# jimonld2000/AudioDenoiser

Measured on AMD Instinct MI355X. Metric: spectrogram frames/sec (forward), 513x256 fp32, higher is better.
Workload: dtype f32; 1 GPU; BASELINE configs[1]: batch=64 synthetic 513x256 fp32 spectrograms on one MI355X, full U-Net forward + per-clip perceptual loss; batch_per_gpu=64, global_batch=64, freq_bins=513, frames=256, parallelism=clips sharded over 1 rank(s), weights replicated, no data-path collective, lib_digest=fdf05542d610

## Files before the change

### audiodenoiser_amd/csrc/adn_internal.h

```cpp
#pragma once
#include <hip/hip_runtime.h>
#include <cstddef>
#include <cstdint>

namespace adn {

template <typename T> constexpr int ACT_BLOCK = 32 / (int)sizeof(T);
template <typename T>
__host__ __device__ __forceinline__ long act_off(int C, long HW, long pix, int c)
{
    constexpr int B = ACT_BLOCK<T>;
    (void)C;
    return ((long)(c / B) * HW + pix) * B + (c % B);
}

#ifdef __HIPCC__
constexpr unsigned ADN_DMA_OOB = 0xfffffff0u;
__device__ __forceinline__ void dma16_buf(__amdgpu_buffer_rsrc_t rsrc, unsigned voff, unsigned soff, float *lds_wave_base)
{
    __builtin_amdgcn_raw_ptr_buffer_load_lds(rsrc, (__attribute__((address_space(3))) void *)lds_wave_base, 16, voff, soff, 0, 0);
}
__device__ __forceinline__ __amdgpu_buffer_rsrc_t dma_rsrc(const void *base, unsigned bytes)
{
    return __builtin_amdgcn_make_buffer_rsrc(const_cast<void *>(base), 0, bytes, 0x00020000);
// ... 50 lines not shown
    void *pool;
    int N, H, W;
    int Cout;
    int tilesY, tilesX, nct;
    int pair;
    FastDiv fdGc, fdNcg, fdTx, fdTy;
    int nwg_total;
    int split;
    int ksplit;
    int nwg_base;
    float *partial;
    const float *dotw;
    float *dot_out;
    float dot_bias;
    const float *firstw, *firstb;
};

inline bool wino4_pair_mode(const ConvArgs &a)
{
    if (a.W > 16) return false;
    const size_t i0 = (size_t)a.s0.C * a.s0.H * a.s0.W * 4, i1 = (size_t)a.s1.C * a.s1.H * a.s1.W * 4;
    return (i0 > i1 ? i0 : i1) + (size_t)a.H * a.W * 32 < (size_t)0xfffffff0u;
}

constexpr int ADN_MAX_KSPLIT = 8;

inline long conv_workgroups(const ConvArgs &a) { return (long)a.N * a.tilesY * a.tilesX * a.nct; }

inline int wino_ksplit(long nwg, int nchunk)
{
// ... 23 lines not shown
        }
    }
    return best;
}

inline int conv16_ksplit(long nwg, int nchunk, size_t out_floats)
{
    if (nwg > 64) return 1;
    int ks = 1;
    while (ks < 8 && nwg * ks * 2 <= 256 && nchunk % (ks * 2) == 0 && nchunk / (ks * 2) >= 4 &&
           (size_t)(ks * 2) * out_floats * 4 <= ((size_t)32 << 20))
        ks *= 2;
    return ks;
}

enum ConvKind { CONV3X3_RELU = 0, CONV3X3_RELU_POOL = 1, CONVT2X2 = 2, CONV3X3_RELU_DOT = 3 };

struct ConvGeom {
    int TH;
    int BN;
    int KC;
};
ConvGeom conv_geom(ConvKind kind, int Cout, bool f16);
long conv_mfma_tiles(ConvKind kind, bool f16, ConvArgs &a);

hipError_t launch_conv_mfma(ConvKind kind, const ConvArgs &a, bool f16, hipStream_t st);
hipError_t launch_conv_reduce_f16(ConvKind kind, const float *partial, const float *bias, void *out, void *pool, int ksplit, int N,
                                  int H, int W, int Cout, hipStream_t st);
hipError_t launch_convt_reduce(const float *partial, const float *bias, float *out, int ksplit, int N, int Ho, int Wo, int Cout,
                               hipStream_t st);
constexpr int WINO_BN = 32;
hipError_t launch_wino_conv(ConvKind kind, const ConvArgs &a, hipStream_t st);
long wino_tiles(ConvArgs &a);
hipError_t launch_wino_reduce(ConvKind kind, const ConvArgs &a, hipStream_t st);
bool wino4_applicable(ConvKind kind, const ConvArgs &a, bool force);
long wino4_workgroups(const ConvArgs &a);
hipError_t launch_wino4_conv(ConvKind kind, const ConvArgs &a, hipStream_t st);

bool conv16_applicable(ConvKind kind, const ConvArgs &a);
hipError_t launch_conv16(ConvKind kind, const ConvArgs &a, bool resident, hipStream_t st);

bool convt16_applicable(const ConvArgs &a);
hipError_t launch_convt16(const ConvArgs &a, hipStream_t st);

hipError_t launch_conv_first(const float *x, const float *w9x64, const float *bias, void *out, bool f16,
                             int N, int H, int W, int Cin, hipStream_t st);
hipError_t launch_dot_finish(const float *planes, int nplanes, float bias, float *y, long npix, hipStream_t st);
hipError_t launch_conv_out(const void *in, bool f16, const float *w64, float bias, float *out, long npix, long HW,
                           long out_stride, hipStream_t st);
hipError_t launch_nhwc_to_nchw(const void *in, bool f16, float *out, int N, int H, int W, int C, hipStream_t st);

hipError_t launch_stft_mag(const float *audio, int n_clips, long L, int n_fft, int hop, int center, long n_frames,
// ... 76 lines not shown
```

### audiodenoiser_amd/csrc/conv_kernels.hip

```cpp
#include "adn_internal.h"

#include <atomic>
#include <cstdlib>

namespace adn {

typedef float f32x16 __attribute__((ext_vector_type(16)));
typedef float f32x4 __attribute__((ext_vector_type(4)));
typedef _Float16 f16x8 __attribute__((ext_vector_type(8)));
typedef _Float16 f16x4 __attribute__((ext_vector_type(4)));

namespace {

constexpr int TW = 16;
constexpr int CONVT_KG = 2, CONVT_WPE = 4;

template <typename T> struct Elem;
template <> struct Elem<float> { static constexpr int EPV = 4; };
template <> struct Elem<_Float16> { static constexpr int EPV = 8; };

__device__ __forceinline__ int xcd_remap(int b, int nwg)
{
    const int xcd = b & 7, q = nwg >> 3, r = nwg & 7;
    const int start = xcd < r ? xcd * (q + 1) : r * (q + 1) + (xcd - r) * q;
// ... 249 lines not shown
template <> struct Piece<_Float16> { typedef f16x8 type; };

template <typename T, int TH, int BN, int WM, int WN, int EPI, int HALVES = 1>
__device__ __forceinline__ void conv_epilogue_staged(const ConvArgs &p, f32x16 (&acc)[TH * TW / 32 / WM][BN / 32 / WN],
                                                     const float (&bias_r)[BN / 32 / WN], float *smem, int tid, int lane,
                                                     int wave, int ct, int n, int ty, int tx)
{
    constexpr int MB = TH * TW / 32 / WM, NB = BN / 32 / WN, NT = 64 * WM * WN;
    constexpr int EPP = 16 / sizeof(T);
    constexpr int RS = BN + EPP;
    constexpr int NPIX = TH * TW, PPR = BN / EPP;
    typedef typename Piece<T>::type piece_t;
    const int wm = wave / WN, wn = wave % WN;
    const int hh = lane >> 5, l31 = lane & 31;
    T *stage = reinterpret_cast<T *>(smem);
    static_assert(HALVES == 1 || (EPI == CONVT2X2 && HALVES == 2 && WM == 2 && TH % 2 == 0), "two-half staging: convT, WM = 2");

#pragma unroll
    for (int hf = 0; hf < HALVES; ++hf) {
    if (HALVES == 1 || wm == hf) {
#pragma unroll
    for (int j = 0; j < NB; ++j) {
        const int col = (wn * NB + j) * 32 + l31;
        const float bv = bias_r[j];
#pragma unroll
        for (int i = 0; i < MB; ++i) {
            const int pix0 = ((HALVES == 1 ? wm * MB : 0) + i) * 32 + 4 * hh;
            float v[16];
#pragma unroll
            for (int r = 0; r < 16; ++r) {
                v[r] = acc[i][j][r] + bv;
                if (EPI != CONVT2X2) v[r] = relu_nan(v[r]);
            }
            if constexpr (sizeof(T) == 4) {
#pragma unroll
                for (int r = 0; r < 16; ++r) stage[(pix0 + (r & 3) + 8 * (r >> 2)) * RS + col] = v[r];
            } else {
                const bool odd = l31 & 1;
#pragma unroll
                for (int r = 0; r < 16; r += 2) {
                    const float send = odd ? v[r] : v[r + 1];
                    const float recv = __shfl_xor(send, 1, 64);
                    const float lo = odd ? recv : v[r], hi = odd ? v[r + 1] : recv;
                    const int pix = pix0 + ((r + (odd ? 1 : 0)) & 3) + 8 * (r >> 2);
                    typedef _Float16 h2 __attribute__((ext_vector_type(2)));
                    *reinterpret_cast<h2 *>(stage + pix * RS + (col & ~1)) = h2{(_Float16)lo, (_Float16)hi};
                }
// ... 10 lines not shown
        const int Ho = 2 * p.H, Wo = 2 * p.W;
        const int ncg = p.Cout >> 6, di = ct / ncg, cg = ct - di * ncg;
        const size_t bstr = (size_t)Ho * Wo * BE;
        T *ob = outp + (size_t)n * Ho * Wo * p.Cout + (size_t)(NBLK * cg) * bstr;
        const int gxl = lane >> 2, dj = (lane >> 1) & 1, half = lane & 1;
        const int gx = tx * TW + gxl;
        constexpr int THH = TH / HALVES;
#pragma unroll
        for (int it = 0; it < NBLK * THH / (NT / 64); ++it) {
            const int run = it * (NT / 64) + wave;
            const int b8 = run / THH, py = run - b8 * THH;
            const int gy = ty * TH + hf * THH + py;
            const piece_t val = *reinterpret_cast<const piece_t *>(stage + (py * TW + gxl) * RS + dj * 64 + b8 * BE + half * EPP);
            if (gy < p.H && gx < p.W)
                *reinterpret_cast<piece_t *>(ob + b8 * bstr + ((size_t)(2 * gy + di) * Wo + 2 * gx + dj) * BE + half * EPP) = val;
        }
        if (HALVES > 1 && hf + 1 < HALVES) __syncthreads();
    } else if constexpr (EPI == CONV3X3_RELU_DOT) {
        static_assert(PPR <= 64 && (PPR & (PPR - 1)) == 0 && NT % PPR == 0, "pieces of a pixel must sit in one wave");
        float wv[EPP];
#pragma unroll
        for (int e = 0; e < EPP; ++e) wv[e] = p.dotw[(tid % PPR) * EPP + e];
#pragma unroll
        for (int it = 0; it < NPIX * PPR / NT; ++it) {
            const int id = it * NT + tid;
            const int pix = id / PPR, part = id - pix * PPR;
            const int gy = ty * TH + (pix >> 4), gx = tx * TW + (pix & 15);
            const piece_t val = *reinterpret_cast<const piece_t *>(stage + pix * RS + part * EPP);
            float s = 0.f;
#pragma unroll
// ... 55 lines not shown
    static constexpr int SLOTS = A_SLOTS + B_SLOTS;
    static constexpr int NPIECE = (SLOTS + NT - 1) / NT;
    static constexpr int A_ROUNDS = (A_SLOTS + NT - 1) / NT;
    static constexpr size_t LDS_BYTES = (size_t)2 * SLOTS * 16;
    static_assert(B_SLOTS % 64 == 0, "weight slab must be a whole number of wave copies");
};

typedef adn_bf16x8 bf16x8;

template <typename T, int TH, int BN, int WM, int WN, int TAPS, int KG, int EPI, int WPE, int SPLIT = 0, int KSPLIT = 0>
__global__ __launch_bounds__(64 * WM * WN, WPE) void conv_dma(const ConvArgs p)
{
    using C = DmaCfg<T, TH, BN, WM, WN, TAPS, KG, SPLIT>;
    static_assert(!KSPLIT || EPI == CONVT2X2 || (sizeof(T) == 2 && EPI == CONV3X3_RELU), "K split: transposed convolutions, fp16 3x3 layers");
    static_assert(!SPLIT || (sizeof(T) == 4 && KG == 2 && TAPS == 1), "SPLIT: fp32 storage, one 16-channel chunk (two fp32 k-groups), 1 tap");
    constexpr int NT = C::NT, EPV = Elem<T>::EPV, HALO = C::HALO, PW = C::PW;
    static_assert(2 * EPV == ACT_BLOCK<T>, "one k-group = one channel block of the activation layout");
    constexpr int PSLOT = C::PSLOT, RSLOT = C::RSLOT, A_SLOTS = C::A_SLOTS, SLOTS = C::SLOTS, NPIECE = C::NPIECE;
    constexpr int A_ROUNDS = C::A_ROUNDS;
    constexpr int B_DW = C::B_SLOTS * 4;
    constexpr int MB = TH * TW / 32 / WM, NB = BN / 32 / WN;
    static_assert(WM * WN == 4 || WM * WN == 8, "4 or 8 waves per workgroup");
    static_assert(MB >= 1 && NB >= 1, "tile too small");

    extern __shared__ __attribute__((aligned(16))) float smem[];

    const int tid = threadIdx.x;
    const int lane = tid & 63;
    const int wave = __builtin_amdgcn_readfirstlane(tid >> 6);
    const int wm = wave / WN, wn = wave % WN;
// ... 12 lines not shown
        ct = lid - q1 * p.nct;
        const int q2 = fastdiv(q1, p.fdTx.d, p.fdTx.m);
        tx = q1 - q2 * p.tilesX;
        n = fastdiv(q2, p.fdTy.d, p.fdTy.m);
        ty = q2 - n * p.tilesY;
    } else {
        ct = lid % p.nct;
        lid /= p.nct;
        tx = lid % p.tilesX;
        lid /= p.tilesX;
        ty = lid % p.tilesY;
        n = lid / p.tilesY;
    }
    const int gy0 = ty * TH - HALO, gx0 = tx * TW - HALO;

    auto src_base = [&](const ConvSrc &s) { return reinterpret_cast<const char *>(static_cast<const T *>(s.ptr) + (size_t)n * s.H * s.W * s.C); };
    const char *hptr = src_base(p.s0);
    const __amdgpu_buffer_rsrc_t wrs = dma_rsrc(static_cast<const float *>(p.wpk) + (size_t)ct * p.nchunk * B_DW,
                                                (unsigned)((size_t)p.nchunk * B_DW * 4));
    unsigned cstr = (unsigned)((size_t)KG * p.s0.H * p.s0.W * ACT_BLOCK<T> * sizeof(T));
    unsigned wsoff = 0;
    const int c0 = KSPLIT ? ksp * nloc : 0;
    bool in2 = false;
    if constexpr (KSPLIT) {
        wsoff = (unsigned)c0 * (unsigned)(B_DW * 4);
        if (c0 > p.nchunk0) {
            in2 = true;
            cstr = (unsigned)((size_t)KG * p.s1.H * p.s1.W * ACT_BLOCK<T> * sizeof(T));
            hptr = src_base(p.s1) + (size_t)(c0 - p.nchunk0) * cstr;
        } else {
            hptr += (size_t)c0 * cstr;
        }
    }
    const unsigned loff = lane * 16;
    unsigned hcur[A_ROUNDS];
// ... 6 lines not shown
        } else if (want_b) {
            dma16_buf(wrs, loff, wsoff + (unsigned)(sb - A_SLOTS) * 16u, dst);
        }
    };
#pragma unroll
    for (int k = 0; k < NPIECE; ++k) dma_piece(k, 0, false, true);

    auto plan = [&](const ConvSrc &src) {
#pragma unroll
        for (int r = 0; r < A_ROUNDS; ++r) {
            const int s = r * NT + tid;
            const int row = s / RSLOT, k = s - row * RSLOT;
            const int pix = k / PSLOT, q = k - pix * PSLOT;
            const bool data = s < C::A_USED && pix < PW && q < C::KQ;
            const int y0 = gy0 + row - src.offY, x0 = gx0 + pix - src.offX;
            hcur[r] = (data && y0 >= 0 && y0 < src.H && x0 >= 0 && x0 < src.W)
                          ? (unsigned)act_off<T>(src.C, (long)src.H * src.W, y0 * src.W + x0, q * EPV) * (unsigned)sizeof(T) : ADN_DMA_OOB;
        }
    };
    if (in2) plan(p.s1);
    else plan(p.s0);

    auto dma_chunk = [&](int c, int buf, bool with_b = true) {
        if (c == p.nchunk0) {
            hptr = src_base(p.s1);
            cstr = (unsigned)((size_t)KG * p.s1.H * p.s1.W * ACT_BLOCK<T> * sizeof(T));
            plan(p.s1);
        }
#pragma unroll
        for (int k = 0; k < NPIECE; ++k) dma_piece(k, buf, true, with_b);
        hptr += cstr;
        wsoff += B_DW * 4;
    };

    float bias_r[NB];
#pragma unroll
    for (int j = 0; j < NB; ++j) bias_r[j] = p.bias[ct * BN + (wn * NB + j) * 32 + l31];

    f32x16 acc[MB][NB];
#pragma unroll
    for (int i = 0; i < MB; ++i)
#pragma unroll
        for (int j = 0; j < NB; ++j)
#pragma unroll
            for (int r = 0; r < 16; ++r) acc[i][j][r] = 0.f;

    const int a_lane = ((wm * MB * 2 + ((lane >> 4) & 1)) * RSLOT + (lane & 15) * PSLOT) * 4 + hh * 4;
    const int b_lane = A_SLOTS * 4 + hh * BN * 4 + (wn * NB * 32 + l31) * 4;

    dma_chunk(c0, 0, false);
    asm volatile("s_waitcnt vmcnt(0)" ::: "memory");
    __syncthreads();
// ... 46 lines not shown
                } else {
#pragma unroll
                    for (int i = 0; i < MB; ++i)
#pragma unroll
                        for (int j = 0; j < NB; ++j)
                            acc[i][j] = __builtin_amdgcn_mfma_f32_32x32x16_f16(__builtin_bit_cast(f16x8, a[i]),
                                                                               __builtin_bit_cast(f16x8, b[j]), acc[i][j], 0, 0, 0);
                }
            }
        }
        asm volatile("s_waitcnt vmcnt(0)" ::: "memory");
        __syncthreads();
    }
    if constexpr (KSPLIT && EPI != CONVT2X2) {
        conv_epilogue_raw<TH, BN, WM, WN>(p, acc, lane, wave, ct, n + ksp * p.N, ty, tx);
    } else if constexpr (sizeof(T) == 2 || EPI == CONVT2X2) {
        constexpr size_t tile = (size_t)TH * TW * (BN + 16 / sizeof(T)) * sizeof(T);
        constexpr int HALVES = tile <= C::LDS_BYTES ? 1 : 2;
        static_assert(tile / HALVES <= C::LDS_BYTES, "staging tile (or half of it) must fit the two images");
        conv_epilogue_staged<T, TH, BN, WM, WN, EPI, HALVES>(p, acc, bias_r, smem, tid, lane, wave, ct, KSPLIT ? n + ksp * p.N : n, ty, tx);
    } else {
        conv_epilogue<T, TH, BN, WM, WN, EPI>(p, acc, bias_r, lane, wave, ct, n, ty, tx);
    }
}

constexpr int FIRST_ROWS = 8;

template <typename T>
__global__ __launch_bounds__(256) void conv_first_kernel(const float *__restrict__ x, const float *__restrict__ w9x64,
                                                         const float *__restrict__ bias, T *__restrict__ out,
                                                         int H, int W, int tiles_y, int tiles_x, int cols, int Cin)
// ... 280 lines not shown

long conv_mfma_tiles(ConvKind kind, bool f16, ConvArgs &a)
{
    const ConvGeom g = conv_geom(kind, a.Cout, f16);
    a.tilesY = (a.H + g.TH - 1) / g.TH;
    a.tilesX = (a.W + TW - 1) / TW;
    a.nct = (kind == CONVT2X2 ? 4 * a.Cout : a.Cout) / g.BN;
    return conv_workgroups(a);
}

hipError_t launch_conv_mfma(ConvKind kind, const ConvArgs &a, bool f16, hipStream_t st)
{
    return f16 ? launch_conv_mfma_t<_Float16>(kind, a, st) : launch_conv_mfma_t<float>(kind, a, st);
}

hipError_t launch_conv_reduce_f16(ConvKind kind, const float *partial, const float *bias, void *out, void *pool, int ksplit, int N,
                                  int H, int W, int Cout, hipStream_t st)
{
    const bool pl = kind == CONV3X3_RELU_POOL;
    const long items = pl ? (long)N * ((H + 1) / 2) * ((W + 1) / 2) * (Cout / 4) : (long)N * H * W * (Cout / 4);
    const long blocks = (items + 255) / 256;
    if (ksplit < 2 || ksplit > ADN_MAX_KSPLIT || (Cout & 15) || (kind != CONV3X3_RELU && !pl) || (pl && !pool) || blocks <= 0 || blocks > 0x7fffffffL)
        return hipErrorInvalidValue;
    if (pl)
        hipLaunchKernelGGL(conv_reduce_f16_kernel<true>, dim3((unsigned)blocks), dim3(256), 0, st, partial, bias,
                           static_cast<_Float16 *>(out), static_cast<_Float16 *>(pool), ksplit, N, H, W, Cout);
    else
        hipLaunchKernelGGL(conv_reduce_f16_kernel<false>, dim3((unsigned)blocks), dim3(256), 0, st, partial, bias,
                           static_cast<_Float16 *>(out), static_cast<_Float16 *>(nullptr), ksplit, N, H, W, Cout);
    return hipGetLastError();
// ... 77 lines not shown
```

### audiodenoiser_amd/csrc/unet.hip

```cpp
#include "adn_host.h"

#include <algorithm>
#include <cmath>
#include <cstdlib>
#include <cstring>
#include <memory>
#include <vector>

using adn::aligned_to;
using adn::DeviceGuard;
using adn::fail;
using adn::fail_hip;

namespace {

constexpr float BN_EPS = 1e-5f;
constexpr int CH[5] = {64, 128, 256, 512, 1024};

enum LayerKind { CONV3, CONVT };
struct LayerDesc {
    LayerKind kind;
    int level;
    int C0, C1;
    int Cout;
// ... 14 lines not shown
        t.v[t.n++] = LayerDesc{CONVT, l + 1, CH[l + 1], 0, CH[l]};
        t.v[t.n++] = LayerDesc{CONV3, l, CH[l], CH[l], CH[l]};
        t.v[t.n++] = LayerDesc{CONV3, l, CH[l], 0, CH[l]};
    }
    return t;
}
constexpr LayerTable NET = make_layers();
static_assert(NET.n == N_LAYERS && NET.v[0].Cout == 64 && NET.v[8].C0 == 1024 && NET.v[9].kind == CONVT && NET.v[N_LAYERS - 1].Cout == 64,
              "layer table: 9 layers down to the bottleneck, then 4 x (convT, conv, conv)");
static_assert(6 * (1 + N_CONV3) + 2 * N_CONVT + 2 == ADN_N_WEIGHT_TENSORS, "layer table does not match the weight tensor list");
static_assert(1 + N_LAYERS + 1 == ADN_N_LAUNCHES, "layer table does not match the timing slots");

struct LayerWeights {
    size_t w_off, b_off;
    size_t w4_off;
    size_t w16_off;
    size_t braw_off;
};

}

struct adn_unet {
    int device = 0;
    float *dev = nullptr;
    size_t dev_floats = 0;
    size_t first_w = 0, first_b = 0;
    LayerWeights lw[N_LAYERS] = {};
    size_t out_w = 0;
    size_t zero_off = 0;
    float out_b = 0.f;
    std::vector<float> out_bias;
    int in_ch = 1, n_classes = 1;
    std::vector<hipEvent_t> events;
    int timing_max = 0, timing_count = 0;
    bool f16 = false;
    bool use_wino = true;
    bool use_wino4 = true, force_wino4 = false;
    bool allow_split = false;
    bool convt_split = true;
    int f16_conv = 1;
    int f16_convt = 1;
    bool f16_fuse_first = true;
    bool batch_invariant = false;
    long auto_grid = 192, auto_grid64 = 512;
};

namespace {

void bn_fold(const float *b, const float *gamma, const float *beta, const float *mean, const float *var, int C,
             std::vector<float> &scale, std::vector<float> &bias)
{
    scale.resize(C);
    bias.resize(C);
    for (int c = 0; c < C; ++c) {
        const float s = gamma[c] / std::sqrt(var[c] + BN_EPS);
        scale[c] = s;
        bias[c] = (b[c] - mean[c]) * s + beta[c];
    }
}
// ... 130 lines not shown
inline uint16_t bf16_rne(float f)
{
    uint32_t u;
    std::memcpy(&u, &f, 4);
    if ((u & 0x7fffffffu) > 0x7f800000u) return (uint16_t)((u >> 16) | 0x40);
    u += 0x7fffu + ((u >> 16) & 1u);
    return (uint16_t)(u >> 16);
}
inline float bf16_to_float(uint16_t b)
{
    const uint32_t u = (uint32_t)b << 16;
    float f;
    std::memcpy(&f, &u, 4);
    return f;
}
void pack_convt_split(const float *w , int Cin, int Cout, uint16_t *dst)
{
    const int BN = 128, KC = 16;
    const int ncol = 4 * Cout, nct = ncol / BN, nchunk = Cin / KC;
    size_t o = 0;
    for (int ct = 0; ct < nct; ++ct)
        for (int ch = 0; ch < nchunk; ++ch)
            for (int plane = 0; plane < 3; ++plane)
                for (int h = 0; h < 2; ++h)
                    for (int n = 0; n < BN; ++n) {
                        int ij, co;
                        convt_column_host(ct * BN + n, Cout, ij, co);
                        for (int kk = 0; kk < 8; ++kk) {
                            const int ci = ch * KC + 8 * h + kk;
                            const float v = w[((size_t)ci * Cout + co) * 4 + ij];
                            uint16_t hi = bf16_rne(v);
                            if ((hi & 0x7fffu) == 0x7f80u && std::isfinite(v)) hi = (uint16_t)((hi & 0x8000u) | 0x7f7fu);
                            const float r1 = v - bf16_to_float(hi);
                            const uint16_t mid = bf16_rne(r1);
                            const float r2 = r1 - bf16_to_float(mid);
                            dst[o++] = plane == 0 ? hi : plane == 1 ? mid : bf16_rne(r2);
                        }
                    }
}


adn::ConvArgs geom_args(const LayerDesc &d, bool f16, bool wino, int N, int H, int W)
{
    const adn::ConvKind kind = d.kind == CONVT ? adn::CONVT2X2 : adn::CONV3X3_RELU;
    adn::ConvArgs a{};
    a.s0.C = d.C0;
    a.s1.C = d.C1;
    a.N = N;
    a.H = H;
    a.W = W;
    a.Cout = d.Cout;
// ... 85 lines not shown
    adn::ConvArgs a = geom_args(d, h->f16, false, p.N, H, W);
    a.s0 = adn::ConvSrc{in, H, W, d.C0, 0, 0};
    a.s1 = adn::ConvSrc{in, 0, 0, 0, 0, 0};
    a.wpk = h->dev + h->lw[i].w_off;
    a.bias = h->dev + h->lw[i].b_off;
    a.out = out;
    a.split = h->convt_split ? 1 : 0;
    return a;
}


enum Conv3Kernel {
    DIRECT,
    CONV16,
    WINO2,
    WINO4
};
struct Conv3Choice {
    Conv3Kernel kernel;
    int ksplit;
    bool fuse_first;
    bool fuse_out;
};

Conv3Choice choose_conv3(const adn_unet *h, adn::ConvKind kind, const adn::ConvArgs &a, bool first = false, bool tail = false)
{
    Conv3Choice c{DIRECT, 1, false, false};
    if (h->f16) {
        const bool c16 = a.wpk4 && adn::conv16_applicable(kind, a);
        c.fuse_out = tail && a.nct == 1;
        if (first && h->f16_fuse_first && c16) {
            c.kernel = CONV16;
            c.fuse_first = true;
            return c;
        }
        if (a.wpk4 && !h->batch_invariant && !c.fuse_out)
            c.ksplit = adn::conv16_ksplit(adn::conv_workgroups(a), a.nchunk, (size_t)a.N * a.H * a.W * a.Cout);
        if (c.ksplit == 1 && c16) c.kernel = CONV16;
        return c;
    }
// ... 3 lines not shown
    auto done = [&]() {
        c.fuse_first = first && c.kernel == WINO2 && c.ksplit == 1;
        return c;
    };
    const bool can_split = !c.fuse_out;
    const bool f4_ok = a.wpk4 && adn::wino4_applicable(kind, a, h->force_wino4);
    const long g2 = adn::conv_workgroups(a);
    if (h->allow_split && can_split) {
        c.ksplit = adn::wino_ksplit(g2, a.nchunk);
        if (c.ksplit == 1 && f4_ok) c.kernel = WINO4;
        return done();
    }
    const bool automatic = !h->batch_invariant && !h->force_wino4;
    const long thr = a.Cout <= 64 ? h->auto_grid64 : h->auto_grid;
    const long g4 = f4_ok ? adn::wino4_workgroups(a) : 0;
    if (f4_ok && (!automatic || g4 >= thr)) {
        c.kernel = WINO4;
        return done();
    }
    if (automatic && can_split) c.ksplit = adn::wino_ksplit(g2, a.nchunk);
    if (automatic && can_split && f4_ok) {
        const int ks4 = adn::wino4_ksplit(g4, a.nchunk);
        if (ks4 > 1) {
            const double out_mb = (double)a.N * a.H * a.W * a.Cout * 4.0 * 1e-6;
            auto reduce_us = [&](int ks) { return ks > 1 ? 4.0 + (ks + 1) * out_mb / 8.0 : 0.0; };
            const double t4 = 12.0 + 2.79 * (a.nchunk / ks4) * (double)((g4 * ks4 + 255) / 256) + reduce_us(ks4);
            const double t2 = 8.0 + 2.06 * (a.nchunk / c.ksplit) * (double)((g2 * c.ksplit + 511) / 512) + reduce_us(c.ksplit);
            if (t4 < t2) {
                c.kernel = WINO4;
                c.ksplit = ks4;
            }
        }
    }
    return done();
}

hipError_t launch_conv3(const adn_unet *h, adn::ConvKind kind, const Conv3Choice &c, adn::ConvArgs a, float *partial, hipStream_t st)
{
    if (c.fuse_out) kind = adn::CONV3X3_RELU_DOT;
    switch (c.kernel) {
    case CONV16:
        a.wpk = a.wpk4;
        a.nchunk0 = a.s0.C / 32;
        a.nchunk = (a.s0.C + a.s1.C) / 32;
        if (c.fuse_first) a.nchunk0 = a.nchunk = 2;
        return adn::launch_conv16(kind, a, c.fuse_first || (a.s0.C + a.s1.C == 64 && a.Cout == 64), st);
    case DIRECT:
        if (c.ksplit > 1) {
            adn::ConvArgs sl = a;
            sl.ksplit = c.ksplit;
            sl.out = partial;
            sl.pool = nullptr;
            hipError_t e = adn::launch_conv_mfma(adn::CONV3X3_RELU, sl, true, st);
            if (e != hipSuccess) return e;
            return adn::launch_conv_reduce_f16(kind, partial, a.bias, a.out, a.pool, c.ksplit, a.N, a.H, a.W, a.Cout, st);
// ... 66 lines not shown
    const bool f16 = h->f16;
    const bool timed = h->timing_max > 0 && h->timing_count < h->timing_max && !taps;
    hipEvent_t *ev = timed ? h->events.data() + (size_t)h->timing_count * (ADN_N_LAUNCHES + 1) : nullptr;
    int evi = 0;
#define ADN_MARK()                                          \
    do {                                                    \
        if (timed) ADN_HIP(hipEventRecord(ev[evi++], st));  \
    } while (0)

    auto export_tap = [&](int idx, const void *buf, int layer) -> hipError_t {
        if (!taps || !taps[idx]) return hipSuccess;
        const LayerDesc &d = NET.v[layer];
        return adn::launch_nhwc_to_nchw(buf, f16, taps[idx], N, p.H[d.level], p.W[d.level], d.Cout, st);
    };
    int i = 0;

    const void *cur = tA;
    for (int l = 0; l < 4; ++l) {
        void *skip = ws + p.skip[l], *pool = ws + p.pool[l];
        if (l > 0) {
            const adn::ConvArgs a = conv_args(h, p, i++, ws + p.pool[l - 1], nullptr, 0, 0, tA, nullptr);
            ADN_MARK();
            ADN_HIP(launch_conv3(h, adn::CONV3X3_RELU, choose_conv3(h, adn::CONV3X3_RELU, a), a, part, st));
        }
        adn::ConvArgs a = conv_args(h, p, i++, cur, nullptr, 0, 0, skip, pool);
        const Conv3Choice c = choose_conv3(h, adn::CONV3X3_RELU_POOL, a, l == 0 && h->in_ch == 1);
        if (l == 0) {
            ADN_MARK();
            if (c.fuse_first) {
                a.s0 = adn::ConvSrc{x, p.H[0], p.W[0], 1, 0, 0};
                a.firstw = h->dev + h->first_w;
                a.firstb = h->dev + h->first_b;
            } else {
                ADN_HIP(adn::launch_conv_first(x, h->dev + h->first_w, h->dev + h->first_b, tA, f16, N, p.H[0], p.W[0], h->in_ch, st));
            }
        }
        ADN_MARK();
        ADN_HIP(launch_conv3(h, adn::CONV3X3_RELU_POOL, c, a, part, st));
        ADN_HIP(export_tap(l, skip, i - 1));
    }
    {
        const adn::ConvArgs a = conv_args(h, p, i++, ws + p.pool[3], nullptr, 0, 0, tA, nullptr);
        ADN_MARK();
        ADN_HIP(launch_conv3(h, adn::CONV3X3_RELU, choose_conv3(h, adn::CONV3X3_RELU, a), a, part, st));
        const adn::ConvArgs b = conv_args(h, p, i++, tA, nullptr, 0, 0, tB, nullptr);
        ADN_MARK();
        ADN_HIP(launch_conv3(h, adn::CONV3X3_RELU, choose_conv3(h, adn::CONV3X3_RELU, b), b, part, st));
        ADN_HIP(export_tap(4, tB, i - 1));
    }
    void *X = tB, *Y = tA;
    Conv3Choice last{};
    for (int l = 3; l >= 0; --l) {
        const LayerWeights &TL = h->lw[i];
        const adn::ConvArgs t = convt_args(h, p, i++, X, Y);
        ADN_MARK();
        ADN_HIP(launch_convt(h, TL, choose_convt(h, TL, t), t, part, st));
        const adn::ConvArgs a = conv_args(h, p, i++, ws + p.skip[l], Y, 2 * t.H, 2 * t.W, X, nullptr);
        ADN_MARK();
        ADN_HIP(launch_conv3(h, adn::CONV3X3_RELU, choose_conv3(h, adn::CONV3X3_RELU, a), a, part, st));
        adn::ConvArgs b = conv_args(h, p, i++, X, nullptr, 0, 0, Y, nullptr);
        last = choose_conv3(h, adn::CONV3X3_RELU, b, false, l == 0 && !taps && h->n_classes == 1);
        if (last.fuse_out) {
            b.dotw = h->dev + h->out_w;
            b.dot_out = f16 ? y : static_cast<float *>(Y);
            if (f16) b.dot_bias = h->out_b;
        }
        ADN_MARK();
        ADN_HIP(launch_conv3(h, adn::CONV3X3_RELU, last, b, part, st));
        ADN_HIP(export_tap(5 + (3 - l), Y, i - 1));
        std::swap(X, Y);
    }
    ADN_MARK();
    if (last.fuse_out && f16) {
    } else if (last.fuse_out)
        ADN_HIP(adn::launch_dot_finish(static_cast<const float *>(X), 2, h->out_b, y, (long)N * F * T, st));
    else
        for (int k = 0; k < h->n_classes; ++k)
            ADN_HIP(adn::launch_conv_out(X, f16, h->dev + h->out_w + (size_t)64 * k, h->out_bias[k], y + (size_t)k * F * T,
                                         (long)N * F * T, (long)F * T, (long)h->n_classes * F * T, st));
    ADN_MARK();
    if (timed) {
        if (evi != ADN_N_LAUNCHES + 1) return fail(ADN_ERR_INVALID, "internal: launch count mismatch");
        ++h->timing_count;
// ... 31 lines not shown

void read_switches(adn_unet &h)
{
    if (const char *algo = std::getenv("ADN_CONV_ALGO"))
        h.use_wino = std::strcmp(algo, "direct") != 0;
    if (h.f16) h.use_wino = false;
    if (const char *sk = std::getenv("ADN_WINO_SPLITK")) h.allow_split = std::atoi(sk) != 0;
    if (const char *cs = std::getenv("ADN_CONVT_SPLIT")) h.convt_split = std::atoi(cs) != 0;
    if (const char *bi = std::getenv("ADN_BATCH_INVARIANT")) h.batch_invariant = std::atoi(bi) != 0;
    if (const char *ff = std::getenv("ADN_F16_FIRST")) h.f16_fuse_first = std::atoi(ff) != 0;
    if (const char *fc = std::getenv("ADN_F16_CONV")) h.f16_conv = std::atoi(fc) == 32 ? 0 : 1;
    if (const char *ft = std::getenv("ADN_F16_CONVT")) h.f16_convt = std::strcmp(ft, "dma") == 0 ? 0 : 1;
    if (const char *ag = std::getenv("ADN_AUTO_GRID")) h.auto_grid = std::atol(ag);
    if (const char *ag = std::getenv("ADN_AUTO_GRID64")) h.auto_grid64 = std::atol(ag);
    if (h.f16) h.convt_split = false;
    if (const char *wt = std::getenv("ADN_WINO_TILE")) {
        h.use_wino4 = std::atoi(wt) != 2;
        h.force_wino4 = std::atoi(wt) == 4;
    }
}

void pack_weights(adn_unet &h, const float *const *t, std::vector<float> &host)
{
    auto reserve = [&](size_t n) {
        const size_t at = host.size();
        host.resize(at + ((n + 63) & ~size_t(63)), 0.f);
        return at;
    };
    auto halfs = [&](size_t off) { return reinterpret_cast<_Float16 *>(host.data() + off); };
    std::vector<float> scale, bias;
// ... 38 lines not shown
            }
            ti += 2;
            continue;
        }
        bn_fold(t[ti + 1], t[ti + 2], t[ti + 3], t[ti + 4], t[ti + 5], Cout, scale, bias);
        if (h.f16 && h.f16_conv != 0 && Cin % 32 == 0 && Cout % 64 == 0) {
            L.w16_off = reserve(n16);
            pack_conv16(t[ti], scale, Cin, Cout, halfs(L.w16_off));
        }
        if (h.use_wino) {
            L.w_off = reserve((size_t)16 * Cin * Cout);
            pack_wino3x3(t[ti], scale, Cin, Cout, adn::WINO_BN, host.data() + L.w_off);
            if (h.use_wino4) {
                L.w4_off = reserve((size_t)36 * Cin * Cout);
                pack_wino4_3x3(t[ti], scale, Cin, Cout, host.data() + L.w4_off);
            }
        } else if (h.f16) {
            L.w_off = reserve(n16);
            pack_conv3x3<_Float16>(t[ti], scale, Cin, Cout, halfs(L.w_off));
        } else {
            L.w_off = reserve((size_t)9 * Cin * Cout);
            pack_conv3x3<float>(t[ti], scale, Cin, Cout, host.data() + L.w_off);
        }
        L.b_off = reserve(Cout);
        std::memcpy(host.data() + L.b_off, bias.data(), sizeof(float) * Cout);
        ti += 6;
    }
    h.zero_off = reserve(4 * 512);
    h.out_w = reserve((size_t)64 * h.n_classes);
    std::memcpy(host.data() + h.out_w, t[ti], sizeof(float) * 64 * h.n_classes);
// ... 125 lines not shown
```

Measured before the change: 491,100 frames/s.

## Add staged Winograd F(4,3) path with batched split-bf16 MFMA GEMM for deep layers

Adds a three-stage Winograd F(4x4,3x3) convolution for the deep fp32 layers (Cin >= 512, level >= 3): an input-transform kernel writes V to scratch, a batched GEMM over the 36 transform points reuses the split-bf16 MFMA DMA kernel with a new WINO_GEMM epilogue, and an output-transform kernel applies bias, ReLU and optional pooling. The aim is to turn these large-channel layers into large, well-occupied MFMA GEMMs and cut the multiply count compared with the fused Winograd and direct kernels. The cost is extra global-memory round trips for the V and M scratch buffers (carved from the unused parts of the activation buffers), two extra launches per layer, and more packed weight memory. The path is taken automatically when the scratch fits and the GEMM grid is large enough.

```diff
diff --git a/audiodenoiser_amd/csrc/adn_internal.h b/audiodenoiser_amd/csrc/adn_internal.h
--- a/audiodenoiser_amd/csrc/adn_internal.h
+++ b/audiodenoiser_amd/csrc/adn_internal.h
@@ -88,6 +88,7 @@
     float *dot_out;
     float dot_bias;
     const float *firstw, *firstb;
+    long rows;
 };
 
 inline bool wino4_pair_mode(const ConvArgs &a)
@@ -141,7 +142,7 @@
     return ks;
 }
 
-enum ConvKind { CONV3X3_RELU = 0, CONV3X3_RELU_POOL = 1, CONVT2X2 = 2, CONV3X3_RELU_DOT = 3 };
+enum ConvKind { CONV3X3_RELU = 0, CONV3X3_RELU_POOL = 1, CONVT2X2 = 2, CONV3X3_RELU_DOT = 3, WINO_GEMM = 4 };
 
 struct ConvGeom {
     int TH;
@@ -163,6 +164,17 @@
 bool wino4_applicable(ConvKind kind, const ConvArgs &a, bool force);
 long wino4_workgroups(const ConvArgs &a);
 hipError_t launch_wino4_conv(ConvKind kind, const ConvArgs &a, hipStream_t st);
+
+struct Wino3sGeom {
+    int tilesY, tilesX;
+    long rows;
+    size_t v_bytes, m_bytes;
+    long gemm_grid;
+};
+bool wino3s_applicable(ConvKind kind, const ConvArgs &a);
+Wino3sGeom wino3s_geom(const ConvArgs &a);
+hipError_t launch_wino3s_conv(ConvKind kind, const ConvArgs &a, float *V, float *M, hipStream_t st);
+hipError_t launch_wino_gemm(const float *V, const void *U, float *M, long rows, int Cin, int Cout, hipStream_t st);
 
 bool conv16_applicable(ConvKind kind, const ConvArgs &a);
 hipError_t launch_conv16(ConvKind kind, const ConvArgs &a, bool resident, hipStream_t st);
diff --git a/audiodenoiser_amd/csrc/conv_kernels.hip b/audiodenoiser_amd/csrc/conv_kernels.hip
--- a/audiodenoiser_amd/csrc/conv_kernels.hip
+++ b/audiodenoiser_amd/csrc/conv_kernels.hip
@@ -287,7 +287,8 @@
     const int wm = wave / WN, wn = wave % WN;
     const int hh = lane >> 5, l31 = lane & 31;
     T *stage = reinterpret_cast<T *>(smem);
-    static_assert(HALVES == 1 || (EPI == CONVT2X2 && HALVES == 2 && WM == 2 && TH % 2 == 0), "two-half staging: convT, WM = 2");
+    static_assert(HALVES == 1 || ((EPI == CONVT2X2 || EPI == WINO_GEMM) && HALVES == 2 && WM == 2 && TH % 2 == 0),
+                  "two-half staging: convT / Winograd GEMM, WM = 2");
 
 #pragma unroll
     for (int hf = 0; hf < HALVES; ++hf) {
@@ -303,7 +304,7 @@
 #pragma unroll
             for (int r = 0; r < 16; ++r) {
                 v[r] = acc[i][j][r] + bv;
-                if (EPI != CONVT2X2) v[r] = relu_nan(v[r]);
+                if (EPI != CONVT2X2 && EPI != WINO_GEMM) v[r] = relu_nan(v[r]);
             }
             if constexpr (sizeof(T) == 4) {
 #pragma unroll
@@ -344,6 +345,20 @@
             const piece_t val = *reinterpret_cast<const piece_t *>(stage + (py * TW + gxl) * RS + dj * 64 + b8 * BE + half * EPP);
             if (gy < p.H && gx < p.W)
                 *reinterpret_cast<piece_t *>(ob + b8 * bstr + ((size_t)(2 * gy + di) * Wo + 2 * gx + dj) * BE + half * EPP) = val;
+        }
+        if (HALVES > 1 && hf + 1 < HALVES) __syncthreads();
+    } else if constexpr (EPI == WINO_GEMM) {
+        static_assert(sizeof(T) == 4 && BN % 8 == 0, "Winograd GEMM: fp32");
+        constexpr int HPIX = NPIX / HALVES;
+        T *ob = outp + (size_t)n * p.rows * p.Cout + (size_t)ct * (BN / 8) * p.rows * 8;
+#pragma unroll
+        for (int it = 0; it < HPIX * PPR / NT; ++it) {
+            const int id = it * NT + tid;
+            const int b8 = id / (2 * HPIX), rem = id - b8 * (2 * HPIX), pix = rem >> 1, half = rem & 1;
+            const long row = (long)ty * NPIX + hf * HPIX + pix;
+            if (row < p.rows)
+                *reinterpret_cast<piece_t *>(ob + ((size_t)b8 * p.rows + row) * 8 + half * 4) =
+                    *reinterpret_cast<const piece_t *>(stage + pix * RS + b8 * 8 + half * 4);
         }
         if (HALVES > 1 && hf + 1 < HALVES) __syncthreads();
     } else if constexpr (EPI == CONV3X3_RELU_DOT) {
@@ -429,6 +444,8 @@
     using C = DmaCfg<T, TH, BN, WM, WN, TAPS, KG, SPLIT>;
     static_assert(!KSPLIT || EPI == CONVT2X2 || (sizeof(T) == 2 && EPI == CONV3X3_RELU), "K split: transposed convolutions, fp16 3x3 layers");
     static_assert(!SPLIT || (sizeof(T) == 4 && KG == 2 && TAPS == 1), "SPLIT: fp32 storage, one 16-channel chunk (two fp32 k-groups), 1 tap");
+    constexpr bool GEMM = EPI == WINO_GEMM;
+    static_assert(!GEMM || (SPLIT && !KSPLIT && TW == 16), "Winograd GEMM stage: split-bf16 form");
     constexpr int NT = C::NT, EPV = Elem<T>::EPV, HALO = C::HALO, PW = C::PW;
     static_assert(2 * EPV == ACT_BLOCK<T>, "one k-group = one channel block of the activation layout");
     constexpr int PSLOT = C::PSLOT, RSLOT = C::RSLOT, A_SLOTS = C::A_SLOTS, SLOTS = C::SLOTS, NPIECE = C::NPIECE;
@@ -471,11 +488,12 @@
     }
     const int gy0 = ty * TH - HALO, gx0 = tx * TW - HALO;
 
-    auto src_base = [&](const ConvSrc &s) { return reinterpret_cast<const char *>(static_cast<const T *>(s.ptr) + (size_t)n * s.H * s.W * s.C); };
+    auto src_hw = [&](const ConvSrc &s) { return GEMM ? (size_t)p.rows : (size_t)s.H * s.W; };
+    auto src_base = [&](const ConvSrc &s) { return reinterpret_cast<const char *>(static_cast<const T *>(s.ptr) + (size_t)n * src_hw(s) * s.C); };
     const char *hptr = src_base(p.s0);
-    const __amdgpu_buffer_rsrc_t wrs = dma_rsrc(static_cast<const float *>(p.wpk) + (size_t)ct * p.nchunk * B_DW,
+    const __amdgpu_buffer_rsrc_t wrs = dma_rsrc(static_cast<const float *>(p.wpk) + (size_t)(GEMM ? n * p.nct + ct : ct) * p.nchunk * B_DW,
                                                 (unsigned)((size_t)p.nchunk * B_DW * 4));
-    unsigned cstr = (unsigned)((size_t)KG * p.s0.H * p.s0.W * ACT_BLOCK<T> * sizeof(T));
+    unsigned cstr = (unsigned)((size_t)KG * src_hw(p.s0) * ACT_BLOCK<T> * sizeof(T));
     unsigned wsoff = 0;
     const int c0 = KSPLIT ? ksp * nloc : 0;
     bool in2 = false;
@@ -512,8 +530,8 @@
             const int pix = k / PSLOT, q = k - pix * PSLOT;
             const bool data = s < C::A_USED && pix < PW && q < C::KQ;
             const int y0 = gy0 + row - src.offY, x0 = gx0 + pix - src.offX;
-            hcur[r] = (data && y0 >= 0 && y0 < src.H && x0 >= 0 && x0 < src.W)
-                          ? (unsigned)act_off<T>(src.C, (long)src.H * src.W, y0 * src.W + x0, q * EPV) * (unsigned)sizeof(T) : ADN_DMA_OOB;
+            hcur[r] = (data && y0 >= 0 && y0 < src.H && x0 >= 0 && x0 < src.W && (!GEMM || (long)y0 * src.W + x0 < p.rows))
+                          ? (unsigned)act_off<T>(src.C, (long)src_hw(src), y0 * src.W + x0, q * EPV) * (unsigned)sizeof(T) : ADN_DMA_OOB;
         }
     };
     if (in2) plan(p.s1);
@@ -533,7 +551,7 @@
 
     float bias_r[NB];
 #pragma unroll
-    for (int j = 0; j < NB; ++j) bias_r[j] = p.bias[ct * BN + (wn * NB + j) * 32 + l31];
+    for (int j = 0; j < NB; ++j) bias_r[j] = GEMM ? 0.f : p.bias[ct * BN + (wn * NB + j) * 32 + l31];
 
     f32x16 acc[MB][NB];
 #pragma unroll
@@ -610,7 +628,7 @@
     }
     if constexpr (KSPLIT && EPI != CONVT2X2) {
         conv_epilogue_raw<TH, BN, WM, WN>(p, acc, lane, wave, ct, n + ksp * p.N, ty, tx);
-    } else if constexpr (sizeof(T) == 2 || EPI == CONVT2X2) {
+    } else if constexpr (sizeof(T) == 2 || EPI == CONVT2X2 || GEMM) {
         constexpr size_t tile = (size_t)TH * TW * (BN + 16 / sizeof(T)) * sizeof(T);
         constexpr int HALVES = tile <= C::LDS_BYTES ? 1 : 2;
         static_assert(tile / HALVES <= C::LDS_BYTES, "staging tile (or half of it) must fit the two images");
@@ -921,6 +939,28 @@
     return f16 ? launch_conv_mfma_t<_Float16>(kind, a, st) : launch_conv_mfma_t<float>(kind, a, st);
 }
 
+hipError_t launch_wino_gemm(const float *V, const void *U, float *M, long rows, int Cin, int Cout, hipStream_t st)
+{
+    if (!V || !U || !M || rows < 1 || rows >= (1L << 25) || Cin < 16 || (Cin & 15) || Cout < 128 || (Cout & 127)) return hipErrorInvalidValue;
+    ConvArgs a{};
+    a.N = 36;
+    a.W = TW;
+    a.H = (int)((rows + TW - 1) / TW);
+    a.rows = rows;
+    a.s0 = ConvSrc{V, a.H, a.W, Cin, 0, 0};
+    a.s1 = ConvSrc{V, 0, 0, 0, 0, 0};
+    a.nchunk0 = a.nchunk = Cin / 16;
+    a.wpk = U;
+    a.out = M;
+    a.Cout = Cout;
+    a.ksplit = 1;
+    a.split = 1;
+    a.tilesY = (a.H + 7) / 8;
+    a.tilesX = 1;
+    a.nct = Cout / 128;
+    return launch_dma_cfg<float, 8, 128, 2, 2, 1, CONVT_KG, WINO_GEMM, 3, 1>(a, st);
+}
+
 hipError_t launch_conv_reduce_f16(ConvKind kind, const float *partial, const float *bias, void *out, void *pool, int ksplit, int N,
                                   int H, int W, int Cout, hipStream_t st)
 {
diff --git a/audiodenoiser_amd/csrc/unet.hip b/audiodenoiser_amd/csrc/unet.hip
--- a/audiodenoiser_amd/csrc/unet.hip
+++ b/audiodenoiser_amd/csrc/unet.hip
@@ -52,6 +52,7 @@
 struct LayerWeights {
     size_t w_off, b_off;
     size_t w4_off;
+    size_t w3_off;
     size_t w16_off;
     size_t braw_off;
 };
@@ -81,6 +82,8 @@
     bool f16_fuse_first = true;
     bool batch_invariant = false;
     long auto_grid = 192, auto_grid64 = 512;
+    int wino_gemm = 1;
+    long gemm_grid = 1536;
 };
 
 namespace {
@@ -241,6 +244,42 @@
     std::memcpy(&f, &u, 4);
     return f;
 }
+inline void split3_host(float v, uint16_t (&t)[3])
+{
+    uint16_t hi = bf16_rne(v);
+    if ((hi & 0x7fffu) == 0x7f80u && std::isfinite(v)) hi = (uint16_t)((hi & 0x8000u) | 0x7f7fu);
+    const float r1 = v - bf16_to_float(hi);
+    const uint16_t mid = bf16_rne(r1);
+    const float r2 = r1 - bf16_to_float(mid);
+    t[0] = hi;
+    t[1] = mid;
+    t[2] = bf16_rne(r2);
+}
+
+void pack_wino4_split(const float *w , const std::vector<float> &scale, int Cin, int Cout, uint16_t *dst)
+{
+    static const double G[6][3] = {{1.0 / 4, 0, 0},           {-1.0 / 6, -1.0 / 6, -1.0 / 6}, {-1.0 / 6, 1.0 / 6, -1.0 / 6},
+                                   {1.0 / 24, 1.0 / 12, 1.0 / 6}, {1.0 / 24, -1.0 / 12, 1.0 / 6}, {0, 0, 1}};
+    const int nct = Cout / 128, nchunk = Cin / 16;
+    for (int co = 0; co < Cout; ++co)
+        for (int ci = 0; ci < Cin; ++ci) {
+            const float *g = w + ((size_t)co * Cin + ci) * 9;
+            double tmp[6][3];
+            for (int x = 0; x < 6; ++x)
+                for (int b = 0; b < 3; ++b)
+                    tmp[x][b] = G[x][0] * g[0 * 3 + b] + G[x][1] * g[1 * 3 + b] + G[x][2] * g[2 * 3 + b];
+            const int ct = co / 128, n = co % 128, ch = ci / 16, hh = (ci % 16) / 8, kk = ci % 8;
+            for (int x = 0; x < 6; ++x)
+                for (int v = 0; v < 6; ++v) {
+                    const float U = (float)((tmp[x][0] * G[v][0] + tmp[x][1] * G[v][1] + tmp[x][2] * G[v][2]) * (double)scale[co]);
+                    uint16_t t[3];
+                    split3_host(U, t);
+                    uint16_t *slab = dst + (((size_t)(6 * x + v) * nct + ct) * nchunk + ch) * (3 * 2 * 128 * 8);
+                    for (int plane = 0; plane < 3; ++plane) slab[((plane * 2 + hh) * 128 + n) * 8 + kk] = t[plane];
+                }
+        }
+}
+
 void pack_convt_split(const float *w , int Cin, int Cout, uint16_t *dst)
 {
     const int BN = 128, KC = 16;
@@ -255,13 +294,9 @@
                         convt_column_host(ct * BN + n, Cout, ij, co);
                         for (int kk = 0; kk < 8; ++kk) {
                             const int ci = ch * KC + 8 * h + kk;
-                            const float v = w[((size_t)ci * Cout + co) * 4 + ij];
-                            uint16_t hi = bf16_rne(v);
-                            if ((hi & 0x7fffu) == 0x7f80u && std::isfinite(v)) hi = (uint16_t)((hi & 0x8000u) | 0x7f7fu);
-                            const float r1 = v - bf16_to_float(hi);
-                            const uint16_t mid = bf16_rne(r1);
-                            const float r2 = r1 - bf16_to_float(mid);
-                            dst[o++] = plane == 0 ? hi : plane == 1 ? mid : bf16_rne(r2);
+                            uint16_t t[3];
+                            split3_host(w[((size_t)ci * Cout + co) * 4 + ij], t);
+                            dst[o++] = t[plane];
                         }
                     }
 }
@@ -377,7 +412,13 @@
     DIRECT,
     CONV16,
     WINO2,
-    WINO4
+    WINO4,
+    WINO3S
+};
+struct WinoScratch {
+    const void *U = nullptr;
+    float *V = nullptr, *M = nullptr;
+    size_t v_bytes = 0, m_bytes = 0;
 };
 struct Conv3Choice {
     Conv3Kernel kernel;
@@ -386,7 +427,8 @@
     bool fuse_out;
 };
 
-Conv3Choice choose_conv3(const adn_unet *h, adn::ConvKind kind, const adn::ConvArgs &a, bool first = false, bool tail = false)
+Conv3Choice choose_conv3(const adn_unet *h, adn::ConvKind kind, const adn::ConvArgs &a, bool first = false, bool tail = false,
+                         const WinoScratch &sc = WinoScratch())
 {
     Conv3Choice c{DIRECT, 1, false, false};
     if (h->f16) {
@@ -420,6 +462,15 @@
     const bool automatic = !h->batch_invariant && !h->force_wino4;
     const long thr = a.Cout <= 64 ? h->auto_grid64 : h->auto_grid;
     const long g4 = f4_ok ? adn::wino4_workgroups(a) : 0;
+    if (h->wino_gemm && sc.U && !c.fuse_out && !first && adn::wino3s_applicable(kind, a)) {
+        const adn::Wino3sGeom g3 = adn::wino3s_geom(a);
+        const bool fits = g3.v_bytes <= sc.v_bytes && g3.m_bytes <= sc.m_bytes;
+        const bool pinned = h->batch_invariant && !h->force_wino4;
+        if (fits && (h->wino_gemm == 2 || pinned || (automatic && g3.gemm_grid >= h->gemm_grid))) {
+            c.kernel = WINO3S;
+            return c;
+        }
+    }
     if (f4_ok && (!automatic || g4 >= thr)) {
         c.kernel = WINO4;
         return done();
@@ -441,10 +492,14 @@
     return done();
 }
 
-hipError_t launch_conv3(const adn_unet *h, adn::ConvKind kind, const Conv3Choice &c, adn::ConvArgs a, float *partial, hipStream_t st)
+hipError_t launch_conv3(const adn_unet *h, adn::ConvKind kind, const Conv3Choice &c, adn::ConvArgs a, float *partial, hipStream_t st,
+                        const WinoScratch &sc = WinoScratch())
 {
     if (c.fuse_out) kind = adn::CONV3X3_RELU_DOT;
     switch (c.kernel) {
+    case WINO3S:
+        a.wpk = sc.U;
+        return adn::launch_wino3s_conv(kind, a, sc.V, sc.M, st);
     case CONV16:
         a.wpk = a.wpk4;
         a.nchunk0 = a.s0.C / 32;
@@ -541,17 +596,32 @@
         return adn::launch_nhwc_to_nchw(buf, f16, taps[idx], N, p.H[d.level], p.W[d.level], d.Cout, st);
     };
     int i = 0;
+    auto wino_scratch = [&](int li) {
+        WinoScratch sc;
+        const LayerDesc &d = NET.v[li];
+        if (f16 || !h->lw[li].w3_off) return sc;
+        const size_t full = (size_t)N * p.H[0] * p.W[0] * 64 * sizeof(float);
+        const size_t front = (size_t)N * p.H[d.level] * p.W[d.level] * std::max(std::max(d.C0, d.C1), d.Cout) * sizeof(float);
+        if (front >= full) return sc;
+        sc.U = h->dev + h->lw[li].w3_off;
+        sc.V = reinterpret_cast<float *>(static_cast<char *>(tA) + front);
+        sc.M = reinterpret_cast<float *>(static_cast<char *>(tB) + front);
+        sc.v_bytes = sc.m_bytes = full - front;
+        return sc;
+    };
 
     const void *cur = tA;
     for (int l = 0; l < 4; ++l) {
         void *skip = ws + p.skip[l], *pool = ws + p.pool[l];
         if (l > 0) {
+            const WinoScratch sc = wino_scratch(i);
             const adn::ConvArgs a = conv_args(h, p, i++, ws + p.pool[l - 1], nullptr, 0, 0, tA, nullptr);
             ADN_MARK();
-            ADN_HIP(launch_conv3(h, adn::CONV3X3_RELU, choose_conv3(h, adn::CONV3X3_RELU, a), a, part, st));
-        }
+            ADN_HIP(launch_conv3(h, adn::CONV3X3_RELU, choose_conv3(h, adn::CONV3X3_RELU, a, false, false, sc), a, part, st, sc));
+        }
+        const WinoScratch sc = wino_scratch(i);
         adn::ConvArgs a = conv_args(h, p, i++, cur, nullptr, 0, 0, skip, pool);
-        const Conv3Choice c = choose_conv3(h, adn::CONV3X3_RELU_POOL, a, l == 0 && h->in_ch == 1);
+        const Conv3Choice c = choose_conv3(h, adn::CONV3X3_RELU_POOL, a, l == 0 && h->in_ch == 1, false, sc);
         if (l == 0) {
             ADN_MARK();
             if (c.fuse_first) {
@@ -563,16 +633,18 @@
             }
         }
         ADN_MARK();
-        ADN_HIP(launch_conv3(h, adn::CONV3X3_RELU_POOL, c, a, part, st));
+        ADN_HIP(launch_conv3(h, adn::CONV3X3_RELU_POOL, c, a, part, st, sc));
         ADN_HIP(export_tap(l, skip, i - 1));
     }
     {
+        const WinoScratch sa = wino_scratch(i);
         const adn::ConvArgs a = conv_args(h, p, i++, ws + p.pool[3], nullptr, 0, 0, tA, nullptr);
         ADN_MARK();
-        ADN_HIP(launch_conv3(h, adn::CONV3X3_RELU, choose_conv3(h, adn::CONV3X3_RELU, a), a, part, st));
+        ADN_HIP(launch_conv3(h, adn::CONV3X3_RELU, choose_conv3(h, adn::CONV3X3_RELU, a, false, false, sa), a, part, st, sa));
+        const WinoScratch sb = wino_scratch(i);
         const adn::ConvArgs b = conv_args(h, p, i++, tA, nullptr, 0, 0, tB, nullptr);
         ADN_MARK();
-        ADN_HIP(launch_conv3(h, adn::CONV3X3_RELU, choose_conv3(h, adn::CONV3X3_RELU, b), b, part, st));
+        ADN_HIP(launch_conv3(h, adn::CONV3X3_RELU, choose_conv3(h, adn::CONV3X3_RELU, b, false, false, sb), b, part, st, sb));
         ADN_HIP(export_tap(4, tB, i - 1));
     }
     void *X = tB, *Y = tA;
@@ -582,18 +654,20 @@
         const adn::ConvArgs t = convt_args(h, p, i++, X, Y);
         ADN_MARK();
         ADN_HIP(launch_convt(h, TL, choose_convt(h, TL, t), t, part, st));
+        const WinoScratch sa = wino_scratch(i);
         const adn::ConvArgs a = conv_args(h, p, i++, ws + p.skip[l], Y, 2 * t.H, 2 * t.W, X, nullptr);
         ADN_MARK();
-        ADN_HIP(launch_conv3(h, adn::CONV3X3_RELU, choose_conv3(h, adn::CONV3X3_RELU, a), a, part, st));
+        ADN_HIP(launch_conv3(h, adn::CONV3X3_RELU, choose_conv3(h, adn::CONV3X3_RELU, a, false, false, sa), a, part, st, sa));
+        const WinoScratch sb = wino_scratch(i);
         adn::ConvArgs b = conv_args(h, p, i++, X, nullptr, 0, 0, Y, nullptr);
-        last = choose_conv3(h, adn::CONV3X3_RELU, b, false, l == 0 && !taps && h->n_classes == 1);
+        last = choose_conv3(h, adn::CONV3X3_RELU, b, false, l == 0 && !taps && h->n_classes == 1, sb);
         if (last.fuse_out) {
             b.dotw = h->dev + h->out_w;
             b.dot_out = f16 ? y : static_cast<float *>(Y);
             if (f16) b.dot_bias = h->out_b;
         }
         ADN_MARK();
-        ADN_HIP(launch_conv3(h, adn::CONV3X3_RELU, last, b, part, st));
+        ADN_HIP(launch_conv3(h, adn::CONV3X3_RELU, last, b, part, st, sb));
         ADN_HIP(export_tap(5 + (3 - l), Y, i - 1));
         std::swap(X, Y);
     }
@@ -655,6 +729,7 @@
     if (const char *ag = std::getenv("ADN_AUTO_GRID")) h.auto_grid = std::atol(ag);
     if (const char *ag = std::getenv("ADN_AUTO_GRID64")) h.auto_grid64 = std::atol(ag);
     if (h.f16) h.convt_split = false;
+    if (const char *wg = std::getenv("ADN_WINO_GEMM")) h.wino_gemm = std::atoi(wg) == 2 ? 2 : std::atoi(wg) != 0;
     if (const char *wt = std::getenv("ADN_WINO_TILE")) {
         h.use_wino4 = std::atoi(wt) != 2;
         h.force_wino4 = std::atoi(wt) == 4;
@@ -723,6 +798,10 @@
             if (h.use_wino4) {
                 L.w4_off = reserve((size_t)36 * Cin * Cout);
                 pack_wino4_3x3(t[ti], scale, Cin, Cout, host.data() + L.w4_off);
+                if (h.wino_gemm && d.level >= 3 && Cin >= 512 && Cin % 16 == 0 && Cout % 128 == 0) {
+                    L.w3_off = reserve((size_t)36 * Cin * Cout * 3 / 2);
+                    pack_wino4_split(t[ti], scale, Cin, Cout, reinterpret_cast<uint16_t *>(host.data() + L.w3_off));
+                }
             }
         } else if (h.f16) {
             L.w_off = reserve(n16);
diff --git a/audiodenoiser_amd/csrc/wino3s_kernels.hip b/audiodenoiser_amd/csrc/wino3s_kernels.hip
--- /dev/null
+++ b/audiodenoiser_amd/csrc/wino3s_kernels.hip
@@ -0,0 +1,170 @@
+#include "adn_internal.h"
+
+namespace adn {
+
+namespace {
+
+typedef float f32x4 __attribute__((ext_vector_type(4)));
+
+__device__ __forceinline__ f32x4 vfma(float c, f32x4 a, f32x4 b) { return __builtin_elementwise_fma(f32x4{c, c, c, c}, a, b); }
+
+__device__ __forceinline__ void bt6v(f32x4 &d0, f32x4 &d1, f32x4 &d2, f32x4 &d3, f32x4 &d4, f32x4 &d5)
+{
+    const f32x4 pe = vfma(-4.f, d2, d4);
+    const f32x4 po = vfma(-4.f, d1, d3);
+    const f32x4 se = d4 - d2;
+    const f32x4 so = d3 - d1;
+    const f32x4 r0 = vfma(4.f, d0, pe) - d2;
+    const f32x4 r5 = vfma(4.f, d1, vfma(-5.f, d3, d5));
+    d0 = r0;
+    d1 = pe + po;
+    d2 = pe - po;
+    d3 = vfma(2.f, so, se);
+    d4 = vfma(-2.f, so, se);
+    d5 = r5;
+}
+__device__ __forceinline__ void at6v(f32x4 m0, f32x4 m1, f32x4 m2, f32x4 m3, f32x4 m4, f32x4 m5, f32x4 &y0, f32x4 &y1, f32x4 &y2,
+                                     f32x4 &y3)
+{
+    const f32x4 a = m1 + m2, b = m1 - m2, c = m3 + m4, d = m3 - m4;
+    y0 = m0 + a + c;
+    y1 = vfma(2.f, d, b);
+    y2 = vfma(4.f, c, a);
+    y3 = vfma(8.f, d, b) + m5;
+}
+
+constexpr int NT = 256;
+
+__global__ __launch_bounds__(NT) void wino3s_input_kernel(const ConvArgs p, float *__restrict__ V, int tilesY, int tilesX, long rows)
+{
+    const long id = (long)blockIdx.x * NT + threadIdx.x;
+    const long row = id >> 1;
+    const int half = (int)(id & 1), cb = blockIdx.y;
+    if (row >= rows) return;
+    const int tx = (int)(row % tilesX);
+    const long r2 = row / tilesX;
+    const int ty = (int)(r2 % tilesY), n = (int)(r2 / tilesY);
+    const bool second = cb >= p.s0.C / 8;
+    const ConvSrc &s = second ? p.s1 : p.s0;
+    const int cbl = second ? cb - p.s0.C / 8 : cb;
+    const float *src = static_cast<const float *>(s.ptr) + ((size_t)n * (s.C / 8) + cbl) * ((size_t)s.H * s.W * 8) + half * 4;
+    const int y0 = 4 * ty - 1 - s.offY, x0 = 4 * tx - 1 - s.offX;
+    f32x4 d[6][6];
+#pragma unroll
+    for (int a = 0; a < 6; ++a)
+#pragma unroll
+        for (int b = 0; b < 6; ++b) {
+            const int y = y0 + a, x = x0 + b;
+            d[a][b] = (y >= 0 && y < s.H && x >= 0 && x < s.W) ? *reinterpret_cast<const f32x4 *>(src + ((size_t)y * s.W + x) * 8)
+                                                                : f32x4{0.f, 0.f, 0.f, 0.f};
+        }
+#pragma unroll
+    for (int a = 0; a < 6; ++a) bt6v(d[a][0], d[a][1], d[a][2], d[a][3], d[a][4], d[a][5]);
+#pragma unroll
+    for (int b = 0; b < 6; ++b) bt6v(d[0][b], d[1][b], d[2][b], d[3][b], d[4][b], d[5][b]);
+    const int ncb = (p.s0.C + p.s1.C) / 8;
+    float *vp = V + ((size_t)cb * rows + row) * 8 + half * 4;
+    const size_t pstr = (size_t)ncb * rows * 8;
+#pragma unroll
+    for (int i = 0; i < 6; ++i)
+#pragma unroll
+        for (int j = 0; j < 6; ++j) *reinterpret_cast<f32x4 *>(vp + (size_t)(6 * i + j) * pstr) = d[i][j];
+}
+
+template <bool POOL>
+__global__ __launch_bounds__(NT) void wino3s_output_kernel(const ConvArgs p, const float *__restrict__ M, int tilesY, int tilesX,
+                                                           long rows)
+{
+    const long id = (long)blockIdx.x * NT + threadIdx.x;
+    const long row = id >> 1;
+    const int half = (int)(id & 1), cb = blockIdx.y;
+    if (row >= rows) return;
+    const int tx = (int)(row % tilesX);
+    const long r2 = row / tilesX;
+    const int ty = (int)(r2 % tilesY), n = (int)(r2 / tilesY);
+    const float *mp = M + ((size_t)cb * rows + row) * 8 + half * 4;
+    const size_t pstr = (size_t)(p.Cout / 8) * rows * 8;
+    f32x4 w[4][6];
+#pragma unroll
+    for (int j = 0; j < 6; ++j) {
+        f32x4 m[6];
+#pragma unroll
+        for (int i = 0; i < 6; ++i) m[i] = *reinterpret_cast<const f32x4 *>(mp + (size_t)(6 * i + j) * pstr);
+        at6v(m[0], m[1], m[2], m[3], m[4], m[5], w[0][j], w[1][j], w[2][j], w[3][j]);
+    }
+    const f32x4 bias = *reinterpret_cast<const f32x4 *>(p.bias + cb * 8 + half * 4);
+    const f32x4 zero = {0.f, 0.f, 0.f, 0.f};
+    f32x4 y[4][4];
+#pragma unroll
+    for (int a = 0; a < 4; ++a) {
+        at6v(w[a][0], w[a][1], w[a][2], w[a][3], w[a][4], w[a][5], y[a][0], y[a][1], y[a][2], y[a][3]);
+#pragma unroll
+        for (int b = 0; b < 4; ++b) y[a][b] = __builtin_elementwise_maximum(y[a][b] + bias, zero);
+    }
+    float *ob = static_cast<float *>(p.out) + ((size_t)n * (p.Cout / 8) + cb) * ((size_t)p.H * p.W * 8) + half * 4;
+#pragma unroll
+    for (int a = 0; a < 4; ++a)
+#pragma unroll
+        for (int b = 0; b < 4; ++b) {
+            const int gy = 4 * ty + a, gx = 4 * tx + b;
+            if (gy < p.H && gx < p.W) *reinterpret_cast<f32x4 *>(ob + ((size_t)gy * p.W + gx) * 8) = y[a][b];
+        }
+    if constexpr (POOL) {
+        const int Hp = p.H >> 1, Wp = p.W >> 1;
+        float *pb = static_cast<float *>(p.pool) + ((size_t)n * (p.Cout / 8) + cb) * ((size_t)Hp * Wp * 8) + half * 4;
+#pragma unroll
+        for (int a = 0; a < 2; ++a)
+#pragma unroll
+            for (int b = 0; b < 2; ++b) {
+                const int py = 2 * ty + a, px = 2 * tx + b;
+                const f32x4 mx = __builtin_elementwise_maximum(__builtin_elementwise_maximum(y[2 * a][2 * b], y[2 * a][2 * b + 1]),
+                                                               __builtin_elementwise_maximum(y[2 * a + 1][2 * b], y[2 * a + 1][2 * b + 1]));
+                if (py < Hp && px < Wp) *reinterpret_cast<f32x4 *>(pb + ((size_t)py * Wp + px) * 8) = mx;
+            }
+    }
+}
+
+}
+
+bool wino3s_applicable(ConvKind kind, const ConvArgs &a)
+{
+    if (kind != CONV3X3_RELU && kind != CONV3X3_RELU_POOL) return false;
+    if (kind == CONV3X3_RELU_POOL && !a.pool) return false;
+    const int Cin = a.s0.C + a.s1.C;
+    if (a.firstw || a.ksplit > 1 || Cin < 16 || (Cin & 15) || (a.s0.C & 7) || a.Cout < 128 || (a.Cout & 127)) return false;
+    return a.N >= 1 && a.H >= 1 && a.W >= 1 && wino3s_geom(a).rows < (1L << 25);
+}
+
+Wino3sGeom wino3s_geom(const ConvArgs &a)
+{
+    Wino3sGeom g{};
+    g.tilesY = (a.H + 3) / 4;
+    g.tilesX = (a.W + 3) / 4;
+    g.rows = (long)a.N * g.tilesY * g.tilesX;
+    g.v_bytes = (size_t)36 * g.rows * (a.s0.C + a.s1.C) * sizeof(float);
+    g.m_bytes = (size_t)36 * g.rows * a.Cout * sizeof(float);
+    g.gemm_grid = 36 * ((g.rows + 127) / 128) * (a.Cout / 128);
+    return g;
+}
+
+hipError_t launch_wino3s_conv(ConvKind kind, const ConvArgs &a, float *V, float *M, hipStream_t st)
+{
+    if (!wino3s_applicable(kind, a) || !V || !M || !a.wpk || !a.bias || !a.out) return hipErrorInvalidValue;
+    const Wino3sGeom g = wino3s_geom(a);
+    const long bx = (2 * g.rows + NT - 1) / NT;
+    const int Cin = a.s0.C + a.s1.C;
+    hipLaunchKernelGGL(wino3s_input_kernel, dim3((unsigned)bx, (unsigned)(Cin / 8)), dim3(NT), 0, st, a, V, g.tilesY, g.tilesX, g.rows);
+    hipError_t e = hipGetLastError();
+    if (e != hipSuccess) return e;
+    e = launch_wino_gemm(V, a.wpk, M, g.rows, Cin, a.Cout, st);
+    if (e != hipSuccess) return e;
+    if (kind == CONV3X3_RELU_POOL)
+        hipLaunchKernelGGL(wino3s_output_kernel<true>, dim3((unsigned)bx, (unsigned)(a.Cout / 8)), dim3(NT), 0, st, a, M, g.tilesY,
+                           g.tilesX, g.rows);
+    else
+        hipLaunchKernelGGL(wino3s_output_kernel<false>, dim3((unsigned)bx, (unsigned)(a.Cout / 8)), dim3(NT), 0, st, a, M, g.tilesY,
+                           g.tilesX, g.rows);
+    return hipGetLastError();
+}
+
+}
```

New measurement: 497,100 frames/s (median of 6 runs). +1.2%, better.
